# Slienteagle-wyb/tdmpc

Measured on AMD Instinct MI355X. Metric: plan-steps/sec (N=512, H=5, iters=6) at 1/2/4/8 MI355X vs CPU ref, higher is better.
Workload: dtype fp32

## Files before the change

tdmpc_amd/csrc/tdmpc_kernels.hip:

```cpp
#include <hip/hip_runtime.h>
#include <hiprand/hiprand_kernel.h>

#include <math.h>
#include <stdint.h>
#include <stdio.h>
#include <stdlib.h>
#include <string.h>
#include <unistd.h>

#include <algorithm>
#include <atomic>
#include <chrono>
#include <mutex>
#include <type_traits>
#include <vector>

#include "../../include/tdmpc_hip.h"

typedef float floatx16 __attribute__((ext_vector_type(16)));

#define DEVI __device__ __forceinline__

#ifdef TDMPC_STAMPS
__device__ unsigned long long* g_stamps;
// ... 227 lines not shown
};

inline int p1_ks(const Layout& w) { return (w.Kx + 31) / 32 <= 4 ? 4 : 6; }
inline int p1_kxs(const Layout& w) { return (int)rup(w.Ap + 32 * p1_ks(w), 16); }

inline P1Region p1_region(const tdmpc_dims* d, const Layout& w) {
    P1Region r;
    memset(&r, 0, sizeof r);
    const size_t T = d->num_samples + d->num_pi, Hm = d->max_horizon;
    size_t o = 0;
    auto take = [&](size_t b) { size_t x = o; o += rup(b, 256); return (unsigned)x; };
    r.o_sync = take(P1_NG * 256 + 256 + 4 * P1_NG * P1_WPG);
    r.xb_t = (unsigned)((size_t)P1_ROWS * p1_kxs(w) * 4);
    r.xb_g = (unsigned)((Hm + 1) * r.xb_t);
    r.o_xb = take((size_t)P1_NG * r.xb_g);
    r.o_h1 = take((size_t)P1_NG * 2 * P1_ROWS * P1_H1LD * 4);
    r.o_zp = take((size_t)P1_NG * 16 * P1_ROWS * w.Lr * 4);
    r.o_rp = take((size_t)P1_NG * 16 * P1_ROWS * 4);
    r.o_pp = take((size_t)P1_NG * 16 * P1_ROWS * w.Ar * 4);
    r.o_qm = take((size_t)P1_NG * 2 * 16 * P1_ROWS * 8);
    r.o_qp = take((size_t)P1_NG * 2 * 16 * P1_ROWS * 4);
    r.o_val = take(2 * T * 4);
    r.o_rl = take(T * 4);
    r.o_mu = take((size_t)P1_NG * P1_ROWS * w.Ap * 4);
    r.o_y2 = take((size_t)P1_NG * 2 * P1_ROWS * P1_H1LD * 4);
    r.total = (unsigned)o;
    return r;
}

__host__ __device__ inline size_t p1_cem_floats(int H, int K, int A, int T) {
    const size_t c = (size_t)(T + 63) / 64 * 64 * 2 + rup((size_t)H * K * A, 4);
    return c > 8192 ? c : 8192;
}
inline size_t p1_lds_bytes(int H, int K, int A, int T) {
    const size_t HA = (size_t)H * A;
    return ((size_t)32 * 3 * 64 * 4 + (size_t)P1_ROWS * 36 + 2 * P1_ROWS + p1_cem_floats(H, K, A, T) +
            3 * rup(HA, 4) + 64 + 64 + 16 + 32 + 648) * 4;
}

inline bool p1_dims_ok(const tdmpc_dims* d, const Layout& w) {
    if (w.M != 512 || d->num_elites > 64) return false;
    const int N = d->num_samples, P = d->num_pi, T = N + P;
    const int sr = (N + P1_NG - 1) / P1_NG, pr = (P + P1_NG - 1) / P1_NG;
    if (sr + pr > P1_ROWS || T > 1024) return false;
    if ((w.Kx + 15) / 16 > 12 || (w.Lp + 15) / 16 > 12 || w.Lr > 128 || w.Ar > 128) return false;
    return p1_lds_bytes(d->max_horizon, d->num_elites, w.A, T) <= 160 * 1024;
}

void make_work(const tdmpc_dims* d, const Layout& w, char* base, Work* k, int extra = 0) {
    const size_t B = d->max_batch, N = d->num_samples, P = d->num_pi, T = N + P + extra, H = d->max_horizon;
    const size_t M = w.M;
    size_t o = 0;
    auto take = [&](size_t bytes) { size_t r = o; o += rup(bytes, 256); return base ? base + r : nullptr; };
    k->xrows = (int)rup(B * T, 32);
    k->x_stride = (size_t)k->xrows * w.Kx;
    k->X = (float*)take((H + 1) * k->x_stride * 4);
    k->H1 = (float*)take((size_t)k->xrows * 2 * M * 4);
    k->H2 = (float*)take((size_t)k->xrows * 2 * M * 4);
    k->st1 = (float2*)take(B * T * (2 * M / 64) * 8);
    k->st2 = (float2*)take(B * T * (2 * M / 64) * 8);
    k->rpart = (float*)take(B * T * (M / 32) * 4);
    k->G = (float*)take(B * T * 4);
    k->rlast = (float*)take(B * T * 4);
    k->value = (float*)take(B * T * 4);
    k->qv = (float*)take(2 * (size_t)k->xrows * 4);
    k->pimu = (float*)take((size_t)k->xrows * w.Ap * 4);
    k->z0c = (float*)take(B * 2 * M * 4);
    k->split_rows = std::min(k->xrows, SPLIT_MAX_ROWS);
    k->zpart = (float*)take((size_t)2 * SPLIT_S * k->split_rows * std::max(w.Lr, w.Ar) * 4);
    k->rpart_s = (float*)take((size_t)2 * SPLIT_S * k->split_rows * 4);
    k->z0 = (float*)take(B * w.Lp * 4);
    k->mean = (float*)take(B * H * w.A * 4);
    k->stdv = (float*)take(B * H * w.A * 4);
    k->enc_tmp = (float*)take(d->modality ? 2 * B * pixel_act_floats(w) * 4 : 256);
    k->p1_bytes = p1_dims_ok(d, w) && !extra ? p1_region(d, w).total : 0;
    k->p1 = k->p1_bytes ? (char*)take(k->p1_bytes) : nullptr;
    k->total = o;
}

size_t cem_lds_bytes(int T, int H, int K, int A) {
    const size_t nl = (T + 63) / 64;
    return nl * 64 * 8 + ((size_t)H * K * A + 64 + 4 * rup((size_t)H * A, 4) + 64 + 32) * 4;
}

bool check_dims(const tdmpc_dims* d) {
    if (!d) return false;
    if (d->num_samples <= 0 || d->num_pi < 0 || d->num_elites <= 0 || d->max_horizon <= 0 ||
        d->max_horizon > 16 || d->max_iterations <= 0 || d->max_batch <= 0) return false;
    const int T = d->num_samples + d->num_pi;
    if (d->num_elites > T || d->num_elites > 64 || T > 4096) return false;
    Layout w;
    if (!make_layout(d, &w)) return false;
    if (w.Kx > 1024 || w.M > 1024 || w.L > 1024 || w.A > 256 || w.E > 1024) return false;
    if (cem_lds_bytes(T, d->max_horizon, d->num_elites, w.A) > 160 * 1024) return false;
    return true;
}

DEVI float elu1(float x) { return x > 0.f ? x : expm1f(x); }
DEVI float fmul(float a, float b) { return __fmul_rn(a, b); }
DEVI float fadd(float a, float b) { return __fadd_rn(a, b); }
DEVI float tclamp(float x, float lo, float hi) { return x != x ? x : fminf(fmaxf(x, lo), hi); }
DEVI float nan_to_num(float x) {
    if (x != x) return 0.f;
    if (isinf(x)) return x > 0 ? 3.402823466e38f : -3.402823466e38f;
    return x;
}
__host__ __device__ inline size_t pidx(size_t r, size_t c, size_t cols) {
    return (r >> 5) * (cols * 32) + (c >> 2) * 128 + (r & 31) * 4 + (c & 3);
}

struct RowMap {
    int G, S, O;
};
DEVI int map_row(const RowMap& r, int m) { return (m / r.G) * r.S + r.O + (m % r.G); }

struct Opnd {
    const float* p; long ts; int q0;
};
struct Outp {
    float* p; long ts; int q0;
};

enum { PRO_PLAIN = 0, PRO_LN_TANH = 1 };
enum { EPI_ELU = 0, EPI_LIN_Z = 1, EPI_PI = 2, EPI_LNSTATS = 3, EPI_ELU_DOT = 4 };

DEVI float elu_f(float x) { return x > 0.f ? x : __expf(x) - 1.f; }
DEVI float tanh_f(float x) {
    const float e = __expf(-2.f * fabsf(x));
    return copysignf(__fdividef(1.f - e, 1.f + e), x);
}

struct LinProb {
    Opnd A; Opnd W;
    const float* bias;
    Outp C;
    int N;
    int nvalid;
    int nstore;
    int epi;
    const float2* ln_stats; int ln_ld; int ln_t0; int ln_nt;
    const float* ln_g; const float* ln_b;
    float2* st_out; int st_ld;
    const float* dotw; float* dot_out; int dot_ld;
};

struct LinArgs {
    LinProb p[2];
    int M, K, kch;
    int a_mapped, c_mapped;
    RowMap amap, cmap;
    int A;
    const float* rpart; int rpart_nt; const float* b3r;
    float* G; float* rlast; float disc; int first, last;
    const float* eps; int eps_G; long eps_env; long eps_off; float min_std, lo, hi;
};

template <int R, int C>
DEVI void lin_epilogue(const LinArgs& args, const LinProb& P, float* smem, int KS, int m0, int n0,
                       const float* sbias, const float* sdotw, const float* srp) {
    constexpr int LDC = C + 4;
    constexpr int BW = C >= 64 ? 64 : C;
    constexpr int NB = C / BW;
    const int nthr = blockDim.x;
    const int epi = P.epi;
    const bool need_red = epi == EPI_LNSTATS || epi == EPI_ELU_DOT;
    {
// ... 1947 lines not shown
#pragma unroll
            for (int k = 0; k < 4; ++k) {
                const int cc = q * 4 + k;
                v[k] = cc < a.A ? tclamp(fadd(mt[cc], fmul(sd[cc], ep[cc])), -1.f, 1.f) : 0.f;
            }
            const int gr = e * a.T + n;
            *(float4*)(a.X + (size_t)t * a.x_stride + (size_t)(gr >> 5) * a.Kx * 32 + (size_t)q * 128 + (gr & 31) * 4) =
                make_float4(v[0], v[1], v[2], v[3]);
        }
    }
}

struct FillArgs {
    float* X; size_t x_stride; int Kx, apq, Tw;
    int B, H, A, Hmax, K;
    int n0, E, mode, eH, mean_row;
    const float* mean; const float* stdv;
    const float* elites;
    const float* eps; long eps_env; long reuse_off;
};

__global__ void __launch_bounds__(256) icem_fill_kernel(const FillArgs a) {
    const int rows = a.E + (a.mean_row ? 1 : 0);
    const long total = (long)a.B * a.H * a.apq * rows;
    for (long it = (long)blockIdx.x * blockDim.x + threadIdx.x; it < total; it += (long)gridDim.x * blockDim.x) {
        long r2 = it;
        const int j = (int)(r2 % rows); r2 /= rows;
        const int q = (int)(r2 % a.apq); r2 /= a.apq;
        const int t = (int)(r2 % a.H);
        const int e = (int)(r2 / a.H);
        const float* mt = a.mean + ((size_t)e * a.Hmax + t) * a.A;
        const float* sd = a.stdv + ((size_t)e * a.Hmax + t) * a.A;
        float v[4];
        int row;
        if (j == a.E) {
            row = 0;
#pragma unroll
            for (int k = 0; k < 4; ++k) v[k] = q * 4 + k < a.A ? mt[q * 4 + k] : 0.f;
        } else {
            row = a.n0 + j;
            const float* el = a.elites + (size_t)e * a.Hmax * a.K * a.A;
#pragma unroll
            for (int k = 0; k < 4; ++k) {
                const int cc = q * 4 + k;
                float x = 0.f;
                if (cc < a.A) {
                    if (a.mode == 2) {
                        x = el[((size_t)t * a.K + j) * a.A + cc];
                    } else if (t < a.eH - 1) {
                        x = el[((size_t)(t + 1) * a.K + j) * a.A + cc];
                    } else {
                        const float ep = a.eps[(size_t)e * a.eps_env + a.reuse_off + ((size_t)t * a.E + j) * a.A + cc];
                        x = tclamp(fadd(mt[cc], fmul(sd[cc], ep)), -1.f, 1.f);
                    }
                }
                v[k] = x;
            }
        }
        const int gr = e * a.Tw + row;
        *(float4*)(a.X + (size_t)t * a.x_stride + (size_t)(gr >> 5) * a.Kx * 32 + (size_t)q * 128 + (gr & 31) * 4) =
            make_float4(v[0], v[1], v[2], v[3]);
    }
}

struct CemArgs {
    int final_iter, iter, H, N, P, T, A, K, Kx, Hmax, I;
    int Tw, NE, pi_base;
    float* elite_store;
    const float* X; size_t x_stride;
    const float* value;
    const float* G; const float* qv; int q_ld; float discH;
    float* value_out;
    const float* rlast;
    float* mean; float* stdv;
    const float* eps; long eps_env; long eps_cem_off; long eps_iter; long eps_act_off;
    const double* u;
    float* prev_mean; int eval_mode;
    float temperature, momentum, omm, std_floor;
    const float* std_floor_p;
    float* action; float* metrics;
    float* elite_out; float* score_out; float* mean_out; float* std_out;
    int no_pick; float* reward_out;
    const int* pstatus; int* status;
};

DEVI uint32_t f2ord(float v) {
    const uint32_t u = __float_as_uint(v);
    return (u & 0x80000000u) ? ~u : (u | 0x80000000u);
}
DEVI float ord2f(uint32_t o) { return __uint_as_float((o & 0x80000000u) ? (o & 0x7fffffffu) : ~o); }
DEVI unsigned long long topk_key(float v, int i) {
    return ((unsigned long long)(~f2ord(v)) << 32) | (unsigned)i;
}
DEVI float key_value(unsigned long long k) { return ord2f(~(uint32_t)(k >> 32)); }

DEVI unsigned long long shfl_xor_u64(unsigned long long v, int m) {
    const unsigned lo = __shfl_xor((unsigned)v, m, 64), hi = __shfl_xor((unsigned)(v >> 32), m, 64);
    return ((unsigned long long)hi << 32) | lo;
}
DEVI unsigned long long wave_sort64(unsigned long long key, int lane) {
    for (int k = 2; k <= 64; k <<= 1)
        for (int j = k >> 1; j > 0; j >>= 1) {
            const unsigned long long o = shfl_xor_u64(key, j);
            const bool up = (lane & k) == 0, lower = (lane & j) == 0;
            key = (lower == up) ? (key < o ? key : o) : (key > o ? key : o);
        }
    return key;
}
DEVI unsigned long long wave_clean64(unsigned long long key, int lane) {
    for (int j = 32; j > 0; j >>= 1) {
        const unsigned long long o = shfl_xor_u64(key, j);
        key = ((lane & j) == 0) ? (key < o ? key : o) : (key > o ? key : o);
    }
    return key;
}
DEVI float wave_sum(float v) {
    for (int off = 32; off > 0; off >>= 1) v += __shfl_xor(v, off, 64);
    return v;
}

DEVI int cem_row(const CemArgs& a, int c) { return c < a.NE ? c : a.pi_base + (c - a.NE); }

__global__ void __launch_bounds__(1024) cem_kernel(const CemArgs a) {
    extern __shared__ __attribute__((aligned(16))) float sm[];
    const int e = blockIdx.x, tid = threadIdx.x, nt = blockDim.x, lane = tid & 63, wave = tid >> 6;
    const int nwv = nt >> 6;
    const int H = a.H, A = a.A, K = a.K, T = a.T, N = a.N;
    const int HA = H * A, HKA = H * K * A;
    const int NL = (T + 63) / 64;
    unsigned long long* key = (unsigned long long*)sm;
    float* EA = (float*)(key + (size_t)NL * 64);
    float* sc = EA + HKA;
    float* omean = sc + 64;
    float* smean = omean + 2 * rup(HA, 4);
    float* sstd = smean + rup(HA, 4);
    int* eidx = (int*)(sstd + rup(HA, 4));
    float* red = (float*)(eidx + 64);
    float* gmean = a.mean + (size_t)e * a.Hmax * A;
    float* gstd = a.stdv + (size_t)e * a.Hmax * A;
    const float* val = a.value + (size_t)e * a.Tw;

    for (int i = tid; i < HA; i += nt) omean[i] = gmean[i];
    for (int l = wave; l < NL; l += nwv) {
        const int i = l * 64 + lane;
        float v = 0.f;
        if (i < T) {
            const int row = cem_row(a, i);
            if (a.qv) {
                const size_t x = (size_t)e * a.Tw + row;
                v = qvalue(a.G[x], a.qv[x], a.qv[a.q_ld + x], a.discH);
                if (a.value_out) a.value_out[((size_t)e * a.I + a.iter) * a.Tw + i] = v;
            } else {
                v = val[row];
                if (a.value_out) a.value_out[((size_t)e * a.I + a.iter) * a.Tw + i] = v;
            }
        }
        const unsigned long long k = i < T ? topk_key(v, i) : ~0ull;
        key[(size_t)l * 64 + lane] = wave_sort64(k, lane);
    }
    __syncthreads();
    for (int stride = 1; stride < NL; stride <<= 1) {
        for (int l = wave * 2 * stride; l < NL; l += nwv * 2 * stride) {
            if (l + stride < NL) {
                const unsigned long long x = key[(size_t)l * 64 + lane];
                const unsigned long long y = key[(size_t)(l + stride) * 64 + 63 - lane];
                key[(size_t)l * 64 + lane] = wave_clean64(x < y ? x : y, lane);
            }
        }
        __syncthreads();
    }
    if (tid < K) eidx[tid] = (int)(key[tid] & 0xffffffffu);
    __syncthreads();
    for (int base = 0; base < HKA; base += 8 * nt) {
        float v[8];
#pragma unroll
        for (int u = 0; u < 8; ++u) {
            const int idx = base + tid + u * nt;
            if (idx < HKA) {
                const int t = idx / (K * A), k = (idx / A) % K, c = idx % A;
                v[u] = a.X[(size_t)t * a.x_stride + pidx((size_t)e * a.Tw + cem_row(a, eidx[k]), c, a.Kx)];
            }
        }
#pragma unroll
        for (int u = 0; u < 8; ++u) {
            const int idx = base + tid + u * nt;
            if (idx < HKA) EA[idx] = v[u];
        }
    }
    if (wave == 0) {
        const float v0 = key_value(key[0]);
        float s = 0.f;
        if (lane < K) s = expf(fmul(a.temperature, key_value(key[lane]) - v0));
        const float tot = wave_sum(s);
        s = lane < K ? __fdiv_rn(s, tot) : 0.f;
        if (lane < 64) sc[lane] = s;
        const float tot2 = wave_sum(s);
        if (lane == 0) red[0] = fadd(tot2, 1e-9f);
    }
    __syncthreads();
    const float den = red[0];
    const float std_floor = a.std_floor_p ? *a.std_floor_p : a.std_floor;
    for (int i = tid; i < HA; i += nt) {
        const int t = i / A, c = i % A;
        const float* ea = EA + (size_t)t * K * A + c;
        float s = 0.f;
        for (int k = 0; k < K; ++k) s = fadd(s, fmul(sc[k], ea[(size_t)k * A]));
        const float mu = __fdiv_rn(s, den);
        float v = 0.f;
        for (int k = 0; k < K; ++k) {
            const float dd = ea[(size_t)k * A] - mu;
            v = fadd(v, fmul(sc[k], fmul(dd, dd)));
        }
        const float sd = tclamp(sqrtf(__fdiv_rn(v, den)), std_floor, 2.f);
        const float nm = fadd(fmul(a.momentum, omean[i]), fmul(a.omm, mu));
        smean[i] = nm; sstd[i] = sd;
        gmean[i] = nm; gstd[i] = sd;
        if (a.mean_out) a.mean_out[((size_t)e * a.I + a.iter) * HA + i] = nm;
        if (a.std_out) a.std_out[((size_t)e * a.I + a.iter) * HA + i] = sd;
    }
    if (a.elite_store)
        for (int i = tid; i < HKA; i += nt) a.elite_store[(size_t)e * a.Hmax * a.K * A + i] = EA[i];
    if (!a.final_iter) return;
    const int pst = a.pstatus ? *a.pstatus : 0;
    if (pst && tid == 0 && a.status)
        __hip_atomic_fetch_or(a.status, pst, __ATOMIC_RELAXED, __HIP_MEMORY_SCOPE_AGENT);
    if (a.elite_out)
        for (int i = tid; i < HKA; i += nt) a.elite_out[(size_t)e * HKA + i] = EA[i];
    if (a.score_out && tid < K) a.score_out[(size_t)e * K + tid] = sc[tid];
    {
        float s = 0.f;
        for (int i = tid; i < T; i += nt) s += a.rlast[(size_t)e * a.Tw + cem_row(a, i)];
        s = wave_sum(s);
        if (lane == 0) red[1 + wave] = s;
    }
    __syncthreads();
    if (a.no_pick) {
        if (tid == 0) {
            float rs = 0.f;
            for (int w = 0; w < nwv; ++w) rs += red[1 + w];
            a.reward_out[e] = rs / (float)T;
        }
        return;
    }
    int* jsel = (int*)(red + 20);
    if (tid == 0) {
        double last = 0.0;
        for (int k = 0; k < K; ++k) last += (double)sc[k];
        const double u = a.u[e];
        double acc = 0.0;
        int j = K - 1;
        for (int k = 0; k < K; ++k) {
            acc += (double)sc[k];
            if (acc / last > u) { j = k; break; }
        }
        *jsel = j;
        float rs = 0.f;
        for (int w = 0; w < nwv; ++w) rs += red[1 + w];
        float cs = 0.f;
        for (int c = 0; c < A; ++c) cs += sstd[c];
        a.metrics[(size_t)e * 2 + 0] = pst ? __builtin_nanf("") : rs / (float)T;
        a.metrics[(size_t)e * 2 + 1] = pst ? __builtin_nanf("") : cs / (float)A;
    }
    __syncthreads();
    const int j = *jsel;
    for (int c = tid; c < A; c += nt) {
        float v = EA[(size_t)j * A + c];
        if (!a.eval_mode) v = fadd(v, fmul(sstd[c], a.eps[(size_t)e * a.eps_env + a.eps_act_off + c]));
        if (pst) v = __builtin_nanf("");
        a.action[(size_t)e * A + c] = v;
        if (a.elite_store) a.elite_store[(size_t)e * a.Hmax * a.K * A + (size_t)j * A + c] = v;
    }
    for (int i = tid; i < HA; i += nt) a.prev_mean[(size_t)e * H * A + i] = smean[i];
}

struct EncArgs {
    const float* x; long x_stride; int xdim;
    int E, L, Lp;
    const float* w1t; const float* b1;
    const float* w2t; const float* b2;
    float* z0;
    float* mean; float* stdv; const float* prev_mean; int warm, H, A, Hmax;
    const int* warm_flags;
    const float* ln_g; const float* ln_b;
    int warm_keep_last;
    float init_std;
};

DEVI void enc_matvec(const float* wt, const float* in, int nin, int nout, float* part, int tid, int nt) {
    const int np = nt / nout > 0 ? nt / nout : 1;
    const int j = tid % nout, p = tid / nout;
    float s = 0.f;
    if (p < np && j < nout) {
#pragma unroll 8
        for (int k = p; k < nin; k += np) s += wt[(size_t)k * nout + j] * in[k];
    }
    if (tid < np * nout) part[tid] = s;
}

__global__ void __launch_bounds__(1024) encode_kernel(const EncArgs a) {
    extern __shared__ __attribute__((aligned(16))) float es[];
    const int e = blockIdx.x, tid = threadIdx.x, nt = blockDim.x;
    float* x = es;
    float* hh = x + rup(a.xdim, 4);
    float* part = hh + rup(a.E, 4);
// ... 819 lines not shown
        a.rpart = c.k.rpart; a.rpart_nt = M / pick_cfg(rows, M, M, 0).bw; a.b3r = c.pw + w.b3r;
        a.G = c.k.G; a.rlast = c.k.rlast; a.disc = disc; a.first = first; a.last = last;
        if ((rc = launch_lin(a, 1, w.L, 0, PRO_PLAIN, c.s))) return rc;
    }
    return 0;
}

int policy(const Ctx& c, int t, int rows, RowMap map, const float* eps, long eps_env, int eps_G, long eps_off,
           float min_std, float* mu_out = nullptr, bool fold = false) {
    const Layout& w = c.w;
    const int M = c.M;
    int rc;
    if (fold && !(use_chain(c, rows, 1, CK_PI) && use_x6(c))) {
        snprintf(g_err, sizeof g_err, "folded pi: chain x6 kernels only");
        return TDMPC_E_DIMS;
    }
    if (use_chain(c, rows, 1, CK_PI)) {
        ChainArgs a = chain0(c, rows, map, t, w.Lp, w.Ap / 4, 1);
        ChainProb& p = a.p[0];
        pi_prob(c, p, a.x6 != 0);
        a.W3 = c.pw + w.wp3; a.b3 = c.pw + w.bp3; a.n3 = w.Ar; a.nvalid = w.A; a.nstore = w.Ap;
        if (a.x6) a.X3 = x6p(c, X6_WP3);
        if (fold) { p.X1 = (const unsigned short*)(c.pw + w.fpi_x6); p.b1 = c.pw + w.fpi_b; }
        a.Xo = Xt(c, t); a.out_q0 = 0;
        a.eps = eps; a.eps_G = eps_G; a.eps_env = eps_env; a.eps_off = eps_off; a.A = w.A;
        a.min_std = min_std; a.lo = (float)(-1.0 + 1e-6); a.hi = (float)(1.0 - 1e-6);
        a.mu_out = mu_out;
        return launch_chain(CH_PI, a, 1, c.s);
    }
    if (use_split_pi(c, rows)) {
        if ((rc = flush_split(c))) return rc;
        SplitArgs a;
        memset(&a, 0, sizeof a);
        a.rows = rows; a.M = M; a.K1 = w.Lp; a.q1 = w.Ap / 4; a.amap = map;
        a.X = Xt(c, t); a.x_ts = (long)c.Kx * 32;
        const bool x6 = use_x6(c) != 0;
        pi_prob(c, a.p[0], x6);
        a.W3 = c.pw + w.wp3; a.n3 = w.Ar;
        if (x6) a.X3 = x6p(c, X6_WP3);
        a.zpart = c.k.zpart; a.rpart = c.k.rpart_s; a.prow = c.k.split_rows;
        if ((rc = launch_split(c, a, 1, x6))) return rc;
        SplitPiArgs f;
        memset(&f, 0, sizeof f);
        f.rows = rows; f.amap = map; f.part = c.k.zpart; f.prow = c.k.split_rows; f.n3 = w.Ar; f.A = w.A;
        f.Ap = w.Ap; f.b3 = c.pw + w.bp3; f.Xo = Xt(c, t); f.x_ts = (long)c.Kx * 32;
        f.eps = eps; f.eps_G = eps_G; f.eps_env = eps_env; f.eps_off = eps_off; f.min_std = min_std;
        f.lo = (float)(-1.0 + 1e-6); f.hi = (float)(1.0 - 1e-6);
        const long nth = (long)rows * (w.Ap / 4);
        hipLaunchKernelGGL(split_pi_finish_kernel, dim3((unsigned)((nth + 255) / 256)), dim3(256), 0, c.s, f);
        HIPCHK(hipGetLastError());
        return 0;
    }
    {
        LinArgs a = args0();
        a.M = rows; a.K = w.Lp; a.a_mapped = 1; a.amap = map;
        LinProb& p = a.p[0];
        p.A = xop(c, t, w.Ap / 4); p.W = wop(c, w.wp1, w.Lp); p.bias = c.pw + w.bp1;
        p.C = hout(c.k.H1, c, 0); p.N = p.nvalid = p.nstore = M; p.epi = EPI_ELU;
        if ((rc = launch_lin(a, 1, M, 0, PRO_PLAIN, c.s))) return rc;
    }
    {
        LinArgs a = args0();
        a.M = rows; a.K = M;
        LinProb& p = a.p[0];
        p.A = hop(c.k.H1, c, 0); p.W = wop(c, w.wp2, M); p.bias = c.pw + w.bp2;
        p.C = hout(c.k.H2, c, 0); p.N = p.nvalid = p.nstore = M; p.epi = EPI_ELU;
        if ((rc = launch_lin(a, 1, M, 0, PRO_PLAIN, c.s))) return rc;
    }
    {
        LinArgs a = args0();
        a.M = rows; a.K = M; a.c_mapped = 1; a.cmap = map;
        LinProb& p = a.p[0];
        p.A = hop(c.k.H2, c, 0); p.W = wop(c, w.wp3, M); p.bias = c.pw + w.bp3;
        p.C = xout(c, t, 0); p.N = w.A; p.nvalid = w.A; p.nstore = w.Ap; p.epi = EPI_PI;
        a.eps = eps; a.eps_G = eps_G; a.eps_env = eps_env; a.eps_off = eps_off; a.A = w.A;
        a.min_std = min_std;
        a.lo = (float)(-1.0 + 1e-6); a.hi = (float)(1.0 - 1e-6);
        return launch_lin(a, 1, w.A, 0, PRO_PLAIN, c.s);
    }
}

int pi_cache_on() {
    static const int v = [] { const char* e = getenv("TDMPC_PI_CACHE"); return e ? atoi(e) : 1; }();
    return v;
}

PiMuArgs pimu_args(const Ctx& c, int rows, RowMap map, const float* eps, long eps_env, int eps_G, long eps_off,
                   float min_std, float* Xo = nullptr, const RowMap* mmap = nullptr) {
    PiMuArgs f;
    memset(&f, 0, sizeof f);
    f.rows = rows; f.amap = map; f.mmap = mmap ? *mmap : map; f.mu = c.k.pimu; f.Ap = c.w.Ap; f.A = c.w.A;
    f.Xo = Xo ? Xo : Xt(c, c.H); f.x_ts = (long)c.Kx * 32;
    f.eps = eps; f.eps_G = eps_G; f.eps_env = eps_env; f.eps_off = eps_off; f.min_std = min_std;
    f.lo = (float)(-1.0 + 1e-6); f.hi = (float)(1.0 - 1e-6);
    return f;
}

int policy_from_mu(const Ctx& c, int rows, RowMap map, const float* eps, long eps_env, int eps_G, long eps_off,
                   float min_std, float* Xo = nullptr, const RowMap* mmap = nullptr) {
    const PiMuArgs f = pimu_args(c, rows, map, eps, eps_env, eps_G, eps_off, min_std, Xo, mmap);
    const long nth = (long)rows * (c.w.Ap / 4);
    if (!nth) return 0;
    hipLaunchKernelGGL(pi_from_mu_kernel, dim3((unsigned)((nth + 255) / 256)), dim3(256), 0, c.s, f);
    HIPCHK(hipGetLastError());
    return 0;
}

int prep_launch(const Ctx& c, const float* noise, int sample_rows, long eps_env, long eps_off, const float* z0,
                const PiMuArgs* pm) {
    PrepArgs a;
    memset(&a, 0, sizeof a);
    a.X = c.k.X; a.x_stride = c.k.x_stride; a.Kx = c.Kx; a.apq = c.w.Ap / 4; a.lpq = c.w.Lp / 4;
    a.B = c.B; a.N = sample_rows; a.T = c.T; a.H = c.H; a.A = c.A;
    a.mean = c.k.mean; a.stdv = c.k.stdv; a.mstride = c.d->max_horizon * c.A;
    a.eps = noise; a.eps_env = eps_env; a.eps_off = eps_off;
    a.z0 = z0;
    a.n_zq = z0 ? (long)c.B * a.lpq * c.T : 0;
    a.n_sq = noise ? (long)c.B * c.H * a.apq * sample_rows : 0;
    if (pm) {
        a.pm = *pm;
        a.n_pm = (long)pm->rows * (pm->Ap / 4);
    }
    const long total = a.n_zq + a.n_sq + a.n_pm;
    if (!total) return 0;
    const int blocks = (int)std::min<long>((total + 255) / 256, 2048);
    hipLaunchKernelGGL(prep_kernel, dim3(blocks), dim3(256), 0, c.s, a);
    HIPCHK(hipGetLastError());
    return 0;
}
int prep(const Ctx& c, const float* noise, int iter, const float* z0, const PiMuArgs* pm = nullptr) {
    return prep_launch(c, noise, c.N, c.eps_env, c.eps_cem_off + (long)iter * c.eps_iter, z0, pm);
}

int q_chain(const Ctx& c, int rows, RowMap map, const float* X = nullptr, float* qo = nullptr, int q_ld = 0,
            bool fold = false) {
    const Layout& w = c.w;
    const int M = c.M;
    ChainArgs a = chain0(c, rows, map, c.H, c.Kx, 0, 2);
    if (X) a.X = X;
    if (fold && !a.x6) {
        snprintf(g_err, sizeof g_err, "folded Q: chain x6 kernels only");
        return TDMPC_E_DIMS;
    }
    for (int q = 0; q < 2; ++q) {
        ChainProb& p = a.p[q];
        p.W1 = c.pw + w.wq1x + (size_t)q * M * c.Kx; p.b1 = c.pw + w.bq1x + q * M;
        p.g1 = c.pw + w.g1 + q * M; p.be1 = c.pw + w.be1 + q * M;
        p.W2 = c.pw + w.wq2 + (size_t)q * M * M; p.b2 = c.pw + w.bq2 + q * M;
        p.g2 = c.pw + w.g2 + q * M; p.be2 = c.pw + w.be2 + q * M;
        p.w3v = c.pw + w.wq3 + q * M; p.b3v = c.pw + w.bq3 + q;
        if (a.x6) {
            p.X1 = x6p(c, X6_WQ1X) + q * x6_w1_rows_stride(c);
            p.X2 = x6p(c, X6_WQ2) + (size_t)q * (M / 32) * (M / 16) * 1536;
        }
        if (fold) {
            p.X1 = (const unsigned short*)(c.pw + w.fq_x6) + q * x6_w1_rows_stride(c);
            p.b1 = c.pw + w.fq_b + q * M;
        }
    }
    a.q = qo ? qo : c.k.qv; a.q_ld = qo ? q_ld : c.k.xrows;
    return launch_chain(CH_Q, a, 2, c.s);
}

int wh_g1p(const Ctx& c) { return (int)rup(c.w.Lp, 32) / 32; }
int wh_nb3p(const Ctx& c) { return (int)rup(c.w.A, 16) / 16; }
int wh_g1q(const Ctx& c) { return (int)rup(c.Kx, 32) / 32; }
// ... 272 lines not shown
    a.u = u; a.prev_mean = prev_mean; a.action = action; a.metrics = metrics;
    a.elite_out = elite_out; a.score_out = score_out; a.value_out = value_out; a.mean_out = mean_out; a.std_out = std_out;
    a.eval_mode = prm->eval_mode; a.min_std = prm->min_std; a.temperature = prm->temperature; a.momentum = prm->momentum;
    a.omm = prm->one_minus_momentum; a.std_floor = prm->std_floor; a.std_floor_p = prm->std_floor_dev;
    for (int t = 0; t <= c.H && t < 17; ++t) a.disc[t] = prm->discount_pow[t];
    a.base = c.k.p1; a.bytes = (unsigned)c.k.p1_bytes;
    a.o_sync = rg.o_sync; a.o_xb = rg.o_xb; a.o_h1 = rg.o_h1; a.o_zp = rg.o_zp; a.o_rp = rg.o_rp; a.o_pp = rg.o_pp;
    a.o_qm = rg.o_qm; a.o_qp = rg.o_qp; a.o_val = rg.o_val; a.o_rl = rg.o_rl; a.o_mu = rg.o_mu; a.o_y2 = rg.o_y2; a.pi_cache = pi_cache_on(); a.xb_t = rg.xb_t; a.xb_g = rg.xb_g;
    a.stamps = g_p1_stamps;
    a.status = prm->status;
    a.pstatus = pack_status(c);
    {
        const char* e = getenv("TDMPC_P1_DEBUG_SKIP");
        a.debug_skip = e && atoi(e) ? 1 : 0;
    }
    hipLaunchKernelGGL(zero_words_kernel, dim3(1), dim3(P1_NG * 64 + 64), 0, c.s, (unsigned*)(c.k.p1 + rg.o_sync),
                       P1_NG * 64 + 64);
    HIPCHK(hipGetLastError());
    const size_t lds = p1_lds_bytes(c.H, a.K, w.A, c.T);
    Profiler& pf = g_prof;
    const bool prof = prof_armed() && pf.cfg == 8;
    if (prof) snprintf(pf.kernel, sizeof pf.kernel, "plan1_kernel<%d>", p1_ks(w));
    HIPCHK(prof_begin(prof, c.s));
#define PLAN1_LAUNCH(KS) \
    if (p1_ks(w) == KS) hipLaunchKernelGGL(plan1_kernel<KS>, dim3(P1_NG * P1_WPG), dim3(P1_NT), lds, c.s, a);
    PLAN1_FOR_EACH(PLAN1_LAUNCH)
#undef PLAN1_LAUNCH
    HIPCHK(hipGetLastError());
    HIPCHK(prof_end(prof, c.s, 0.0));
    return 0;
}

int setup_ctx(Ctx& c, const tdmpc_dims* d, const void* packed, void* ws, size_t ws_bytes, int batch, int H,
              int I, hipStream_t s, int extra_rows = 0) {
    if (!check_dims(d)) { snprintf(g_err, sizeof g_err, "bad dims"); return TDMPC_E_DIMS; }
    c.d = d;
    make_layout(d, &c.w);
    Work probe;
    make_work(d, c.w, nullptr, &probe, extra_rows);
    if (ws_bytes < probe.total) { snprintf(g_err, sizeof g_err, "workspace too small"); return TDMPC_E_SIZE; }
    make_work(d, c.w, (char*)ws, &c.k, extra_rows);
    c.pw = (const float*)packed; c.s = s;
    c.B = batch; c.N = d->num_samples; c.P = d->num_pi; c.T = c.N + c.P; c.H = H; c.path = TDMPC_PATH_AUTO;
    c.A = c.w.A; c.M = c.w.M; c.Kx = c.w.Kx;
    const long A = c.A;
    c.eps_cem_off = (long)H * c.P * A;
    c.eps_iter = (long)H * c.N * A + (long)c.T * A;
    c.eps_term_off = (long)H * c.N * A;
    c.eps_act_off = c.eps_cem_off + (long)I * c.eps_iter;
    c.eps_env = c.eps_act_off + A;
    if (batch <= 0 || batch > d->max_batch || H <= 0 || H > d->max_horizon || I <= 0 || I > d->max_iterations) {
        snprintf(g_err, sizeof g_err, "bad call params");
        return TDMPC_E_DIMS;
    }
    return init_attrs();
}

int resolve_path(int path, bool whole_plan) {
    if (path < 0 || path > TDMPC_PATH_WIDE) { snprintf(g_err, sizeof g_err, "bad path"); return -1; }
    if (path == TDMPC_PATH_CHAIN64) return TDMPC_PATH_CHAIN_X6;
    return path == TDMPC_PATH_PERSIST && !whole_plan ? TDMPC_PATH_AUTO : path;
}

int load_z0(const Ctx& c, const float* z0) {
    const int L = c.w.L;
    hipLaunchKernelGGL(zero_words_kernel, dim3(1), dim3(256), 0, c.s, (unsigned*)c.k.z0, (int)((size_t)c.B * c.w.Lp));
    HIPCHK(hipGetLastError());
    HIPCHK(hipMemcpy2DAsync(c.k.z0, c.w.Lp * 4, z0, L * 4, L * 4, c.B, hipMemcpyDeviceToDevice, c.s));
    return prep(c, nullptr, 0, c.k.z0);
}

template <class Prm>
CemArgs cem_args(const Ctx& c, const Prm* prm, const float* eps, const double* u, float* prev_mean, float* action,
                 float* metrics, float* value_out, float* mean_out, float* std_out) {
    CemArgs ca;
    memset(&ca, 0, sizeof ca);
    ca.H = c.H; ca.N = c.N; ca.P = c.P; ca.T = ca.Tw = ca.NE = c.T; ca.A = c.A; ca.K = c.d->num_elites; ca.Kx = c.Kx;
    ca.Hmax = c.d->max_horizon; ca.mean = c.k.mean; ca.stdv = c.k.stdv; ca.pstatus = pack_status(c);
    ca.X = c.k.X; ca.x_stride = c.k.x_stride; ca.value = c.k.value; ca.rlast = c.k.rlast;
    ca.eps = eps; ca.u = u; ca.prev_mean = prev_mean;
    ca.eval_mode = prm->eval_mode; ca.temperature = prm->temperature; ca.momentum = prm->momentum;
    ca.omm = prm->one_minus_momentum; ca.std_floor = prm->std_floor; ca.action = action; ca.metrics = metrics;
    ca.value_out = value_out; ca.mean_out = mean_out; ca.std_out = std_out; ca.status = prm->status;
    return ca;
}
void cem_args_qv(CemArgs& ca, const Ctx& c, float discH) {
    ca.G = c.k.G; ca.qv = c.k.qv; ca.q_ld = c.k.xrows; ca.discH = discH;
}

struct ToldStep {
    const Ctx& c;
    int operator()(int t, int rows, RowMap map, float disc, int first, int last, int defer) const {
        return step_next(c, t, rows, map, disc, first, last, defer);
    }
};

struct PlanFast {
    bool z0c;
    bool fold;
    bool wide_heads;
    bool pi_cache;
};

template <class Step>
int cem_run(Ctx& c, const Step& step, const PlanFast& f, const tdmpc_plan_params* prm, const float* noise,
            const double* u, float* prev_mean, float* action, float* metrics, float* elite_out, float* score_out,
            float* value_out, float* mean_out, float* std_out) {
    int rc;
    const int H = c.H, I = prm->iterations, B = c.B, N = c.N, P = c.P, T = c.T;
    if ((rc = prep(c, noise, 0, c.k.z0))) return rc;
    if (f.z0c) {
        if ((rc = z0c_launch(c))) return rc;
        c.z0c_ready = 1;
    }
    if (f.fold) {
        const RowMap rm0 = {N, T, 0};
        c.fold_ok = c.w.fold && H > 1 && use_wide(c, B * N, rm0, c.z0c_ready != 0) && use_wide(c, B * N, rm0, false);
        c.fold_heads = c.fold_ok && !f.wide_heads && use_x6(c) && use_chain(c, B * N, 1, CK_PI) &&
                       use_chain(c, B * N, 2, CK_Q) && (P == 0 || use_chain(c, B * P, 2, CK_Q));
        if (c.fold_heads && P > 0 && use_chain(c, B * P, 2, CK_STEP) && use_chain(c, B * P, 1, CK_PI)) {
            const ChainArgs probe = chain0(c, B * P, RowMap{P, T, N}, 0, c.Kx, 0, 2);
            c.fold_policy = probe.rb == 32 && probe.x6;
        }
    }

    const RowMap all = {T, T, 0}, pm = {P, T, N}, rm = {N, T, 0};
    if (P > 0) {
        for (int t = 0; t < H; ++t) {
            if ((rc = policy(c, t, B * P, pm, noise, c.eps_env, P, (long)t * P * c.A, prm->min_std, nullptr,
                             c.fold_policy && t >= 1)))
                return rc;
            if ((rc = step(t, B * T, all, prm->discount_pow[t], t == 0, t == H - 1, 0))) return rc;
        }
    }
    CemArgs ca = cem_args(c, prm, noise, u, prev_mean, action, metrics, value_out, mean_out, std_out);
    ca.I = I; ca.std_floor_p = prm->std_floor_dev; ca.elite_out = elite_out; ca.score_out = score_out;
    ca.eps_env = c.eps_env; ca.eps_cem_off = c.eps_cem_off; ca.eps_iter = c.eps_iter; ca.eps_act_off = c.eps_act_off;
    if (f.wide_heads || c.fold_heads || use_chain(c, B * T, 2, CK_Q)) cem_args_qv(ca, c, prm->discount_pow[H]);
    const size_t cem_lds = cem_lds_bytes(T, H, ca.K, c.A);

    const bool pi_cache = f.pi_cache && P > 0 && use_chain(c, B * T, 1, CK_PI);
    for (int i = 0; i < I; ++i) {
        const long toff = c.eps_cem_off + (long)i * c.eps_iter + c.eps_term_off;
        if (i > 0) {
            const PiMuArgs pmu = pimu_args(c, B * P, pm, noise, c.eps_env, P, toff + (long)N * c.A, prm->min_std);
            if ((rc = prep(c, noise, i, nullptr, f.wide_heads && P > 0 ? &pmu : nullptr))) return rc;
        }
        if (i > 0 || P == 0)
            for (int t = 0; t < H; ++t)
                if ((rc = step(t, B * N, rm, prm->discount_pow[t], t == 0, t == H - 1, 1))) return rc;
        if (f.wide_heads) {
            if (P > 0) {
                if (i == 0) rc = policy(c, H, B * P, pm, noise, c.eps_env, P, toff + (long)N * c.A, prm->min_std, c.k.pimu);
                if (rc || (rc = flush_split(c))) return rc;
            }
            if ((rc = terminal_wide(c, noise, toff, prm->min_std))) return rc;
        } else if (c.fold_heads) {
            if ((rc = policy(c, H, B * N, rm, noise, c.eps_env, N, toff, prm->min_std, nullptr, true))) return rc;
            if (P > 0) {
                if (i == 0 || !pi_cache)
                    rc = policy(c, H, B * P, pm, noise, c.eps_env, P, toff + (long)N * c.A, prm->min_std,
                                pi_cache ? c.k.pimu : nullptr, c.fold_policy != 0);
                else
                    rc = policy_from_mu(c, B * P, pm, noise, c.eps_env, P, toff + (long)N * c.A, prm->min_std);
                if (rc) return rc;
            }
            if ((rc = q_chain(c, B * N, rm, nullptr, nullptr, 0, true))) return rc;
            if (P > 0 && (rc = q_chain(c, B * P, pm, nullptr, nullptr, 0, c.fold_policy != 0))) return rc;
        } else if (pi_cache && i > 0) {
            if ((rc = policy(c, H, B * N, rm, noise, c.eps_env, N, toff, prm->min_std))) return rc;
            if ((rc = flush_split(c))) return rc;
            if ((rc = policy_from_mu(c, B * P, pm, noise, c.eps_env, P, toff + (long)N * c.A, prm->min_std)))
                return rc;
        } else if ((rc = policy(c, H, B * T, all, noise, c.eps_env, T, toff, prm->min_std,
                                pi_cache ? c.k.pimu : nullptr))) {
            return rc;
        }
        if (!f.wide_heads && !c.fold_heads && (rc = terminal_q(c, prm->discount_pow[H]))) return rc;
        ca.final_iter = i == I - 1;
        ca.iter = i;
        hipLaunchKernelGGL(cem_kernel, dim3(B), dim3(1024), cem_lds, c.s, ca);
        HIPCHK(hipGetLastError());
    }
    return 0;
}

bool icem_counts_ok(const tdmpc_icem_params* prm, const tdmpc_dims* d, const char* who) {
    const int H = prm->horizon, I = prm->iterations, N = d->num_samples, K = d->num_elites, P0 = prm->n_pi0;
    if (I <= 0 || I > 16) { snprintf(g_err, sizeof g_err, "%s: 1..16 iterations", who); return false; }
    if (P0 <= 0 || P0 > d->num_pi || prm->n_samples[0] != N) {
        snprintf(g_err, sizeof g_err, "%s: bad counts", who);
        return false;
    }
    for (int i = 0; i < I; ++i) {
        const int Ni = prm->n_samples[i], Pi = prm->n_pi[i], Ei = prm->n_elite[i];
        if (Ni <= 0 || Ni > N || Pi <= 0 || Pi > P0 || Ei < 0 || Ei > K || Ni + Ei + Pi < K ||
            (Ei > 0 && i == 0 && !prm->has_elites) ||
            (i == 0 && Ei > 0 && prm->elite_horizon != H && prm->elite_horizon != H - 1)) {
            snprintf(g_err, sizeof g_err, "%s: bad counts at iteration %d", who, i);
            return false;
        }
    }
    return true;
}

int icem_fill(const Ctx& c, const tdmpc_icem_params* prm, const float* noise, const float* elites, int i) {
    const int last = i == prm->iterations - 1, Ei = prm->n_elite[i];
    if (Ei <= 0 && !last) return 0;
    FillArgs fa;
    memset(&fa, 0, sizeof fa);
    fa.X = c.k.X; fa.x_stride = c.k.x_stride; fa.Kx = c.Kx; fa.apq = c.w.Ap / 4; fa.Tw = c.T;
    fa.B = c.B; fa.H = c.H; fa.A = c.A; fa.Hmax = c.d->max_horizon; fa.K = c.d->num_elites;
    fa.n0 = prm->n_samples[i]; fa.E = Ei; fa.mode = i == 0 ? 1 : 2; fa.eH = prm->elite_horizon; fa.mean_row = last;
    fa.mean = c.k.mean; fa.stdv = c.k.stdv; fa.elites = elites;
    fa.eps = noise; fa.eps_env = prm->env_stride; fa.reuse_off = prm->reuse_off;
    const long tot = (long)c.B * c.H * fa.apq * (Ei + fa.mean_row);
    hipLaunchKernelGGL(icem_fill_kernel, dim3((int)std::min<long>((tot + 255) / 256, 2048)), dim3(256), 0, c.s, fa);
    HIPCHK(hipGetLastError());
    return 0;
}

template <class Step>
int icem_run(Ctx& c, const Step& step, const tdmpc_icem_params* prm, const float* noise, const double* u,
             float* prev_mean, float* elites, float* action, float* metrics, float* value_out, float* mean_out,
             float* std_out) {
    int rc;
    const int H = c.H, I = prm->iterations, B = c.B, K = c.d->num_elites;
    const int Tw = c.d->num_samples + K + c.d->num_pi, pi_base = c.d->num_samples + K, P0 = prm->n_pi0;
    const long A = c.A, env = prm->env_stride;
    c.T = Tw;
    const RowMap pm0 = {P0, Tw, pi_base};
    if ((rc = prep(c, nullptr, 0, c.k.z0))) return rc;
    for (int t = 0; t < H; ++t) {
        if ((rc = policy(c, t, B * P0, pm0, noise, env, P0, prm->pi_off + (long)t * P0 * A, prm->min_std))) return rc;
        if ((rc = step(t, B * P0, pm0, prm->discount_pow[t], t == 0, t == H - 1, 0))) return rc;
    }
    CemArgs ca = cem_args(c, prm, noise, u, prev_mean, action, metrics, value_out, mean_out, std_out);
    ca.I = I; ca.pi_base = pi_base; ca.eps_env = env; ca.eps_act_off = prm->act_off; ca.elite_store = elites;
    cem_args_qv(ca, c, prm->discount_pow[H]);
    const size_t cem_lds = cem_lds_bytes(Tw, H, K, c.A);
    for (int i = 0; i < I; ++i) {
        const int Ni = prm->n_samples[i], Pi = prm->n_pi[i], NE = Ni + prm->n_elite[i];
        if ((rc = prep_launch(c, noise, Ni, env, prm->samp_off[i], nullptr, nullptr))) return rc;
        if ((rc = icem_fill(c, prm, noise, elites, i))) return rc;
        const RowMap blk = {NE, Tw, 0};
        for (int t = 0; t < H; ++t)
            if ((rc = step(t, B * NE, blk, prm->discount_pow[t], t == 0, t == H - 1, 1))) return rc;
        const RowMap pmi = {Pi, Tw, pi_base};
        if ((rc = policy(c, H, B * NE, blk, noise, env, NE, prm->term_off[i], prm->min_std))) return rc;
        if ((rc = policy(c, H, B * Pi, pmi, noise, env, Pi, prm->term_off[i] + (long)NE * A, prm->min_std))) return rc;
        const bool qchain = use_chain(c, B * NE, 2, CK_Q) && use_chain(c, B * Pi, 2, CK_Q);
        if ((rc = terminal_q_rows(c, B * NE, blk, prm->discount_pow[H], qchain))) return rc;
        if ((rc = terminal_q_rows(c, B * Pi, pmi, prm->discount_pow[H], qchain))) return rc;
        ca.qv = qchain ? c.k.qv : nullptr;
        ca.N = Ni; ca.P = Pi; ca.T = NE + Pi; ca.NE = NE;
        ca.final_iter = i == I - 1;
        ca.iter = i;
        hipLaunchKernelGGL(cem_kernel, dim3(B), dim3(1024), cem_lds, c.s, ca);
        HIPCHK(hipGetLastError());
    }
    return 0;
}

template <class Step>
// ... 418 lines not shown
```

Baseline: 6322.

## Fuse next-iteration action sampling into CEM kernel with double-buffered LDS staging

The CEM kernel now also builds the next iteration's sampled action tensor (mean + std*eps, clamped) and the policy-mu items. It streams eps through a register-prefetched, double-buffered LDS tile, which removes the separate prep launch between iterations. The elite gather is rewritten to read float4 vectors directly in the packed X layout, using one wave per elite lane set. The change adds LDS pressure and a serial per-block loop over stages, and only B blocks do the work, which may limit parallelism compared with the separate prep kernel.

```diff
diff --git a/tdmpc_amd/csrc/tdmpc_kernels.hip b/tdmpc_amd/csrc/tdmpc_kernels.hip
--- a/tdmpc_amd/csrc/tdmpc_kernels.hip
+++ b/tdmpc_amd/csrc/tdmpc_kernels.hip
@@ -333,6 +333,15 @@
     const size_t nl = (T + 63) / 64;
     return nl * 64 * 8 + ((size_t)H * K * A + 64 + 4 * rup((size_t)H * A, 4) + 64 + 32) * 4;
 }
+constexpr int CEM_PF = 12;
+int cem_stage_rows(int T, int H, int K, int A, int N) {
+    const size_t base = cem_lds_bytes(T, H, K, A);
+    if (base >= 160 * 1024 || N <= 0) return 0;
+    const size_t floats = std::min<size_t>((160 * 1024 - base) / 8, (size_t)CEM_PF * 1024);
+    int r = (int)std::min<size_t>(N, floats / A);
+    if (r >= 64) r &= ~63;
+    return r;
+}
 
 bool check_dims(const tdmpc_dims* d) {
     if (!d) return false;
@@ -2446,7 +2455,20 @@
     float* elite_out; float* score_out; float* mean_out; float* std_out;
     int no_pick; float* reward_out;
     const int* pstatus; int* status;
+    int fuse, apq, st_rows; float* Xw; long eps_next_off;
+    PiMuArgs pm; int pm_items;
+    unsigned long long* stamps;
 };
+
+#ifdef CEM_STAMPS
+#define CEM_STAMP(k)                                                                                      \
+    do {                                                                                                  \
+        if (a.stamps && blockIdx.x == 0 && threadIdx.x == 0)                                              \
+            a.stamps[1600 + a.iter * 16 + (k)] = __builtin_amdgcn_s_memtime();                            \
+    } while (0)
+#else
+#define CEM_STAMP(k) do {} while (0)
+#endif
 
 DEVI uint32_t f2ord(float v) {
     const uint32_t u = __float_as_uint(v);
@@ -2485,12 +2507,39 @@
 
 DEVI int cem_row(const CemArgs& a, int c) { return c < a.NE ? c : a.pi_base + (c - a.NE); }
 
+struct CemStage { int t, r0, rows; const float* src; };
+DEVI CemStage cem_stage(const CemArgs& a, int e, int s) {
+    const int nch = (a.N + a.st_rows - 1) / a.st_rows;
+    CemStage st;
+    st.t = s / nch;
+    st.r0 = (s - st.t * nch) * a.st_rows;
+    st.rows = min(a.st_rows, a.N - st.r0);
+    st.src = a.eps + (size_t)e * a.eps_env + a.eps_next_off + ((size_t)st.t * a.N + st.r0) * a.A;
+    return st;
+}
+DEVI void cem_stage_load(const CemArgs& a, int e, int s, int nst, int tid, int nt, float (&pf)[CEM_PF]) {
+    if (s >= nst) return;
+    const CemStage st = cem_stage(a, e, s);
+    const int cnt = st.rows * a.A;
+#pragma unroll
+    for (int u = 0; u < CEM_PF; ++u) pf[u] = st.src[min(tid + u * nt, cnt - 1)];
+}
+DEVI void cem_stage_store(const CemArgs& a, int e, int s, int tid, int nt, const float (&pf)[CEM_PF], float* buf) {
+    const int cnt = cem_stage(a, e, s).rows * a.A;
+#pragma unroll
+    for (int u = 0; u < CEM_PF; ++u) {
+        const int idx = tid + u * nt;
+        if (idx < cnt) buf[idx] = pf[u];
+    }
+}
+
 __global__ void __launch_bounds__(1024) cem_kernel(const CemArgs a) {
     extern __shared__ __attribute__((aligned(16))) float sm[];
     const int e = blockIdx.x, tid = threadIdx.x, nt = blockDim.x, lane = tid & 63, wave = tid >> 6;
     const int nwv = nt >> 6;
     const int H = a.H, A = a.A, K = a.K, T = a.T, N = a.N;
     const int HA = H * A, HKA = H * K * A;
+    CEM_STAMP(0);
     const int NL = (T + 63) / 64;
     unsigned long long* key = (unsigned long long*)sm;
     float* EA = (float*)(key + (size_t)NL * 64);
@@ -2498,12 +2547,19 @@
     float* omean = sc + 64;
     float* smean = omean + 2 * rup(HA, 4);
     float* sstd = smean + rup(HA, 4);
-    int* eidx = (int*)(sstd + rup(HA, 4));
-    float* red = (float*)(eidx + 64);
+    float* red = sstd + rup(HA, 4) + 64;
+    float* stg = red + 32;
     float* gmean = a.mean + (size_t)e * a.Hmax * A;
     float* gstd = a.stdv + (size_t)e * a.Hmax * A;
     const float* val = a.value + (size_t)e * a.Tw;
 
+    const int stg_floats = a.st_rows * A;
+    const int nst = a.fuse ? H * ((N + a.st_rows - 1) / a.st_rows) : 0;
+    float pf[CEM_PF];
+    if (a.fuse) {
+        for (int j = tid; j < a.pm_items; j += nt) pi_from_mu_item(a.pm, (long)e * a.pm_items + j);
+        cem_stage_load(a, e, 0, nst, tid, nt, pf);
+    }
     for (int i = tid; i < HA; i += nt) omean[i] = gmean[i];
     for (int l = wave; l < NL; l += nwv) {
         const int i = l * 64 + lane;
@@ -2512,16 +2568,21 @@
             const int row = cem_row(a, i);
             if (a.qv) {
                 const size_t x = (size_t)e * a.Tw + row;
-                v = qvalue(a.G[x], a.qv[x], a.qv[a.q_ld + x], a.discH);
-                if (a.value_out) a.value_out[((size_t)e * a.I + a.iter) * a.Tw + i] = v;
+                const float g = a.G[x], q1 = a.qv[x], q2 = a.qv[a.q_ld + x];
+                v = qvalue(g, q1, q2, a.discH);
             } else {
                 v = val[row];
-                if (a.value_out) a.value_out[((size_t)e * a.I + a.iter) * a.Tw + i] = v;
             }
+            if (a.value_out) a.value_out[((size_t)e * a.I + a.iter) * a.Tw + i] = v;
         }
         const unsigned long long k = i < T ? topk_key(v, i) : ~0ull;
         key[(size_t)l * 64 + lane] = wave_sort64(k, lane);
     }
+    if (nst > 0) {
+        cem_stage_store(a, e, 0, tid, nt, pf, stg);
+        cem_stage_load(a, e, 1, nst, tid, nt, pf);
+    }
+    CEM_STAMP(1);
     __syncthreads();
     for (int stride = 1; stride < NL; stride <<= 1) {
         for (int l = wave * 2 * stride; l < NL; l += nwv * 2 * stride) {
@@ -2533,22 +2594,31 @@
         }
         __syncthreads();
     }
-    if (tid < K) eidx[tid] = (int)(key[tid] & 0xffffffffu);
-    __syncthreads();
-    for (int base = 0; base < HKA; base += 8 * nt) {
-        float v[8];
-#pragma unroll
-        for (int u = 0; u < 8; ++u) {
-            const int idx = base + tid + u * nt;
-            if (idx < HKA) {
-                const int t = idx / (K * A), k = (idx / A) % K, c = idx % A;
-                v[u] = a.X[(size_t)t * a.x_stride + pidx((size_t)e * a.Tw + cem_row(a, eidx[k]), c, a.Kx)];
+    CEM_STAMP(2);
+    {
+        const int npair = H * a.apq, gw = nwv > 1 ? wave - 1 : 0, ngw = nwv > 1 ? nwv - 1 : 1;
+        const size_t erow = lane < K ? (size_t)e * a.Tw + cem_row(a, (int)(key[lane] & 0xffffffffu)) : 0;
+        const float* xe = a.X + (erow >> 5) * ((size_t)a.Kx * 32) + (erow & 31) * 4;
+        for (int p0 = gw >= 0 ? gw : npair; p0 < npair; p0 += 2 * ngw) {
+            float4 v[2];
+            int tt[2], qq[2];
+#pragma unroll
+            for (int u = 0; u < 2; ++u) {
+                const int pr = p0 + u * ngw;
+                tt[u] = pr / a.apq;
+                qq[u] = pr - tt[u] * a.apq;
+                if (pr < npair && lane < K) v[u] = *(const float4*)(xe + (size_t)tt[u] * a.x_stride + (size_t)qq[u] * 128);
             }
-        }
-#pragma unroll
-        for (int u = 0; u < 8; ++u) {
-            const int idx = base + tid + u * nt;
-            if (idx < HKA) EA[idx] = v[u];
+#pragma unroll
+            for (int u = 0; u < 2; ++u) {
+                if (p0 + u * ngw < npair && lane < K) {
+                    float* d = EA + ((size_t)tt[u] * K + lane) * A + 4 * qq[u];
+                    const float vv[4] = {v[u].x, v[u].y, v[u].z, v[u].w};
+#pragma unroll
+                    for (int cc = 0; cc < 4; ++cc)
+                        if (4 * qq[u] + cc < A) d[cc] = vv[cc];
+                }
+            }
         }
     }
     if (wave == 0) {
@@ -2562,15 +2632,18 @@
         if (lane == 0) red[0] = fadd(tot2, 1e-9f);
     }
     __syncthreads();
+    CEM_STAMP(3);
     const float den = red[0];
     const float std_floor = a.std_floor_p ? *a.std_floor_p : a.std_floor;
     for (int i = tid; i < HA; i += nt) {
         const int t = i / A, c = i % A;
         const float* ea = EA + (size_t)t * K * A + c;
         float s = 0.f;
+#pragma unroll 16
         for (int k = 0; k < K; ++k) s = fadd(s, fmul(sc[k], ea[(size_t)k * A]));
         const float mu = __fdiv_rn(s, den);
         float v = 0.f;
+#pragma unroll 16
         for (int k = 0; k < K; ++k) {
             const float dd = ea[(size_t)k * A] - mu;
             v = fadd(v, fmul(sc[k], fmul(dd, dd)));
@@ -2584,6 +2657,39 @@
     }
     if (a.elite_store)
         for (int i = tid; i < HKA; i += nt) a.elite_store[(size_t)e * a.Hmax * a.K * A + i] = EA[i];
+    CEM_STAMP(4);
+    if (nst > 0) {
+        __syncthreads();
+        for (int s = 0; s < nst; ++s) {
+            if (s + 1 < nst) {
+                cem_stage_store(a, e, s + 1, tid, nt, pf, stg + (size_t)((s + 1) & 1) * stg_floats);
+                cem_stage_load(a, e, s + 2, nst, tid, nt, pf);
+            }
+            const CemStage st = cem_stage(a, e, s);
+            const float* tile = stg + (size_t)(s & 1) * stg_floats;
+            const float* mt = smean + st.t * A;
+            const float* sd = sstd + st.t * A;
+            float* xt = a.Xw + (size_t)st.t * a.x_stride;
+            const int R = st.rows, nitems = a.apq * R, dq = nt / R, dn = nt - dq * R;
+            int q = tid / R, n = tid - q * R;
+            for (int it = tid; it < nitems; it += nt) {
+                const float* ep = tile + (size_t)n * A;
+                float v[4];
+#pragma unroll
+                for (int k = 0; k < 4; ++k) {
+                    const int cc = q * 4 + k;
+                    v[k] = cc < A ? tclamp(fadd(mt[cc], fmul(sd[cc], ep[cc])), -1.f, 1.f) : 0.f;
+                }
+                const int gr = e * a.Tw + st.r0 + n;
+                *(float4*)(xt + (size_t)(gr >> 5) * a.Kx * 32 + (size_t)q * 128 + (gr & 31) * 4) =
+                    make_float4(v[0], v[1], v[2], v[3]);
+                q += dq; n += dn;
+                if (n >= R) { n -= R; ++q; }
+            }
+            __syncthreads();
+        }
+        CEM_STAMP(5);
+    }
     if (!a.final_iter) return;
     const int pst = a.pstatus ? *a.pstatus : 0;
     if (pst && tid == 0 && a.status)
@@ -3569,6 +3675,11 @@
 
 int pi_cache_on() {
     static const int v = [] { const char* e = getenv("TDMPC_PI_CACHE"); return e ? atoi(e) : 1; }();
+    return v;
+}
+
+int cem_fused_on() {
+    static const int v = [] { const char* e = getenv("TDMPC_CEM_FUSED"); return e ? atoi(e) : 1; }();
     return v;
 }
 
@@ -4007,6 +4118,8 @@
     ca.eval_mode = prm->eval_mode; ca.temperature = prm->temperature; ca.momentum = prm->momentum;
     ca.omm = prm->one_minus_momentum; ca.std_floor = prm->std_floor; ca.action = action; ca.metrics = metrics;
     ca.value_out = value_out; ca.mean_out = mean_out; ca.std_out = std_out; ca.status = prm->status;
+    ca.apq = c.w.Ap / 4; ca.Xw = c.k.X;
+    ca.stamps = g_p1_stamps;
     return ca;
 }
 void cem_args_qv(CemArgs& ca, const Ctx& c, float discH) {
@@ -4065,9 +4178,12 @@
     const size_t cem_lds = cem_lds_bytes(T, H, ca.K, c.A);
 
     const bool pi_cache = f.pi_cache && P > 0 && use_chain(c, B * T, 1, CK_PI);
+    ca.st_rows = cem_stage_rows(T, H, ca.K, c.A, N);
+    const bool fused = cem_fused_on() && noise && ca.st_rows > 0;
+    const size_t cem_lds_fused = cem_lds + (fused ? 2 * (size_t)ca.st_rows * c.A * 4 : 0);
     for (int i = 0; i < I; ++i) {
         const long toff = c.eps_cem_off + (long)i * c.eps_iter + c.eps_term_off;
-        if (i > 0) {
+        if (i > 0 && !fused) {
             const PiMuArgs pmu = pimu_args(c, B * P, pm, noise, c.eps_env, P, toff + (long)N * c.A, prm->min_std);
             if ((rc = prep(c, noise, i, nullptr, f.wide_heads && P > 0 ? &pmu : nullptr))) return rc;
         }
@@ -4104,7 +4220,16 @@
         if (!f.wide_heads && !c.fold_heads && (rc = terminal_q(c, prm->discount_pow[H]))) return rc;
         ca.final_iter = i == I - 1;
         ca.iter = i;
-        hipLaunchKernelGGL(cem_kernel, dim3(B), dim3(1024), cem_lds, c.s, ca);
+        ca.fuse = fused && i + 1 < I;
+        if (ca.fuse) {
+            ca.eps_next_off = c.eps_cem_off + (long)(i + 1) * c.eps_iter;
+            ca.pm_items = 0;
+            if (f.wide_heads && P > 0) {
+                ca.pm = pimu_args(c, B * P, pm, noise, c.eps_env, P, toff + c.eps_iter + (long)N * c.A, prm->min_std);
+                ca.pm_items = P * (c.w.Ap / 4);
+            }
+        }
+        hipLaunchKernelGGL(cem_kernel, dim3(B), dim3(1024), ca.fuse ? cem_lds_fused : cem_lds, c.s, ca);
         HIPCHK(hipGetLastError());
     }
     return 0;
```

Measured after the change: 6300. Within noise of the previous version (-0.4%).
